# PixelClear/OclPathTracer

Hardware: NVIDIA B200
Metric: Mrays/sec (primary+secondary) (higher is better)
Workload: dtype f32

## Files before the change

oclpathtracer_b200/csrc/capi.cu:

```cuda
#include <cmath>
#include <cstdarg>
#include <cstdio>
#include <cstdlib>
#include <cstring>
#include <map>
#include <memory>
#include <string>
#include <vector>

#include "host_internal.h"
#include "pt_kernels.cuh"
#include "pt_wavefront.cuh"
#include "lbvh.cuh"

namespace ptb {

static thread_local char g_err[512] = "";

int fail(int code, const char* fmt, ...) {
    va_list ap;
    va_start(ap, fmt);
    vsnprintf(g_err, sizeof g_err, fmt, ap);
    va_end(ap);
    return code;
// ... 596 lines not shown
}

extern "C" int ptb_scene_mode_width(ptb_scene* s, int mode) {
    if (!s) return 0;
    const int c = mode_class(s, mode);
    return c == ptd::PTD_FLAT ? 1 : c == ptd::PTD_SMALL4 ? 4 : 2;
}

static ptd::SceneDev scene_dev(const ptb_scene* s, int cls) {
    ptd::SceneDev d;
    d.nodes = s->cls == ptd::PTD_LARGE ? reinterpret_cast<const float4*>(s->d_nodesq) : s->d_nodes;
    d.tris = s->d_tris; d.tris_orig = s->d_tris_orig; d.mats = s->d_mats;
    for (int a = 0; a < 3; ++a) { d.q_lo[a] = s->q_lo[a]; d.q_step[a] = s->q_step[a]; }
    d.n_nodes = s->n_nodes; d.n_tris = s->n_tris; d.n_mats = s->n_mats;
    if (cls == ptd::PTD_SMALL4 && s->cls == ptd::PTD_FLAT) {
        d.nodes = s->d_nodes4; d.n_nodes = int(s->built().nodes4.size());
        d.smem_nodes = s->built().smem_nodes4; d.small = 1; d.flat_n = 0; d.lstack = 0; d.ld256 = 0;
        d.stack_depth = 3 * s->built().depth4 + 1;
        return d;
    }
    const int cap = s->dev->tune[4] > 0 ? s->dev->tune[4] : 0;
    d.smem_nodes = s->small ? s->bfs_nodes : (s->bfs_nodes < cap ? s->bfs_nodes : cap);
    d.small = s->small ? 1 : 0;
    d.flat_n = 0;
    if (s->cls == ptd::PTD_FLAT) {
        d.flat_n = (int(s->built().flat.size()) + 1) & ~1;
        d.smem_nodes = 0;
    }
    d.stack_depth = s->width == 4 ? 3 * s->depth + 1 : s->depth + 1;
    d.lstack = (!s->small && s->dev->tune[2] != 2 && s->depth + 1 <= PTD_LSTACK_ENTRIES) ? 1 : 0;
    d.ld256 = s->dev->tune[8] == 1 ? 0 : 1;
    return d;
}


template <class K>
static int set_smem(K kernel, size_t smem, int block, int* per_sm = nullptr) {
    if (smem > 48 * 1024) CU_TRY(cudaFuncSetAttribute(kernel, cudaFuncAttributeMaxDynamicSharedMemorySize, (int)smem));
    int n = 0;
    CU_TRY(cudaOccupancyMaxActiveBlocksPerMultiprocessor(&n, kernel, block, smem));
    if (n < 1) n = 1;
    const size_t want = size_t(n) * (smem + 1024);
    int pct = (int)((want * 100 + 228 * 1024 - 1) / (228 * 1024));
    if (pct > 100) pct = 100;
    CU_TRY(cudaFuncSetAttribute(kernel, cudaFuncAttributePreferredSharedMemoryCarveout, pct));
    if (per_sm) *per_sm = n;
    return PTB_OK;
}

template <int MODE, bool BVH, int SMALL, bool STATS>
static int launch_mega_t(ptb_device* dev, const ptd::SceneDev& sc, const ptd::RenderArgs& a) {
    const int block = (a.tune[3] == 64 || a.tune[3] == 32) ? a.tune[3] : 128;
    if (MODE == PTB_MODE_PATH && a.tune[5] != 1) {
        const size_t smem = ptd::scene_smem_bytes(sc, BVH, SMALL, block) + (a.tune[9] > 0 ? size_t(a.tune[9]) * 1024 : 0);
        bool state_machine = BVH && SMALL == ptd::PTD_LARGE;
        if (a.tune[5] == 2) state_machine = false;
        if (a.tune[5] == 3) state_machine = BVH;
        const long long total = (long long)a.frames_in_batch * a.n_local;
        const long long need = (total + block - 1) / block;
        unsigned long long* work = dev->counters + 32;
        CU_TRY(cudaMemsetAsync(work, 0, sizeof(unsigned long long), dev->stream));
        int per_sm = 0;
        if constexpr (BVH) {
            if (state_machine) {
                ptd::SceneDev sc2 = sc;
                if (SMALL == ptd::PTD_LARGE && a.tune[4] == 0) sc2.smem_nodes = 0;
                const size_t smem2 = ptd::scene_smem_bytes(sc2, BVH, SMALL, block) + (a.tune[9] > 0 ? size_t(a.tune[9]) * 1024 : 0);
                auto k = ptd::k_path_sm<SMALL, STATS, 0, SMALL == ptd::PTD_LARGE ? 6 : 1>;
                if constexpr (SMALL == ptd::PTD_LARGE && !STATS) {
                    k = ptd::k_path_sm<SMALL, STATS, 8, 6>;
                    if (a.tune[12] == 1) k = ptd::k_path_sm<SMALL, STATS, 0, 6>;
                    if (a.tune[12] == 9) k = ptd::k_path_sm<SMALL, STATS, 9, 6>;
                    if (a.tune[14] == 1) k = ptd::k_path_sm<SMALL, STATS, 8, 1>;
                    if (a.tune[14] == 2) k = ptd::k_path_sm<SMALL, STATS, 8, 2>;
                    if (a.tune[14] == 4) k = ptd::k_path_sm<SMALL, STATS, 8, 4>;
                }
                if constexpr (SMALL == ptd::PTD_LARGE) {
                    if (a.tune[12] != 1 && a.tune[12] != 9 && a.tune[14] == 0 && sc2.lstack && sc2.smem_nodes == 0 && total < (1ll << 31) && a.tune[9] <= 0 && block == 128) {
                        auto k2 = ptd::k_path_sm2<STATS, STATS ? 0 : 11, 6>;
                        if constexpr (!STATS) {
                            if (a.tune[12] == 28) k2 = ptd::k_path_sm2<false, 8, 6>;
                            if (a.tune[12] == 29) k2 = ptd::k_path_sm2<false, 9, 6>;
                            if (a.tune[12] == 30) k2 = ptd::k_path_sm2<false, 10, 6>;
                            if (a.tune[12] == 32) k2 = ptd::k_path_sm2<false, 10, 4>;
                            if (a.tune[12] == 33) k2 = ptd::k_path_sm2<false, 10, 8>;
                        }
                        ptd::RenderArgs a2 = a;
                        if (a2.tune[0] <= 0) a2.tune[0] = 4;
                        if (a2.tune[10] <= 0) a2.tune[10] = 20;
                        if (a2.tune[11] <= 0) a2.tune[11] = 10;
                        const size_t sm2 = ptd::path_sm2_smem_bytes(block);
                        if (int rc = set_smem(k2, sm2, block, &per_sm)) return rc;
                        long long grid2 = (long long)per_sm * dev->prop.multiProcessorCount;
                        if (grid2 > need) grid2 = need;
                        k2<<<(unsigned)grid2, block, sm2, dev->stream>>>(sc2, a2, work);
                        CU_TRY(cudaGetLastError());
                        return PTB_OK;
                    }
                }
                if (int rc = set_smem(k, smem2, block, &per_sm)) return rc;
                if (a.tune[9] < 0 && -a.tune[9] < per_sm) per_sm = -a.tune[9];
                long long grid = (long long)per_sm * dev->prop.multiProcessorCount;
                if (grid > need) grid = need;
                k<<<(unsigned)grid, block, smem2, dev->stream>>>(sc2, a, work);
                CU_TRY(cudaGetLastError());
                return PTB_OK;
            }
        }
        auto k = ptd::k_mega_path_regen<BVH, SMALL, STATS>;
        if constexpr (BVH && SMALL == ptd::PTD_FLAT) if (a.tune[13] != 2) k = ptd::k_mega_path_regen<BVH, SMALL, STATS, true>;
        if (int rc = set_smem(k, smem, block, &per_sm)) return rc;
        long long grid = (long long)per_sm * dev->prop.multiProcessorCount;
        if (grid > need) grid = need;
        k<<<(unsigned)grid, block, smem, dev->stream>>>(sc, a, work);
        CU_TRY(cudaGetLastError());
        return PTB_OK;
    }
    const long long total = (long long)a.frames_in_batch * a.n_local;
    const unsigned grid = (unsigned)((total + block - 1) / block);
    const size_t smem = ptd::scene_smem_bytes(sc, BVH, SMALL, block);
    auto k = ptd::k_mega<MODE, BVH, SMALL, STATS>;
    if (int rc = set_smem(k, smem, block)) return rc;
    k<<<grid, block, smem, dev->stream>>>(sc, a);
    CU_TRY(cudaGetLastError());
    return PTB_OK;
}

template <int MODE>
static int launch_mega_m(ptb_device* dev, const ptd::SceneDev& sc, const ptd::RenderArgs& a, bool bvh, int small, bool stats) {
    using namespace ptd;
    if (!bvh && small == PTD_FLAT) small = PTD_SMALL4;
#define PTB_CASE(B, S, T) if (bvh == B && small == S && stats == T) return launch_mega_t<MODE, B, S, T>(dev, sc, a)
    PTB_CASE(true, PTD_FLAT, false); PTB_CASE(true, PTD_FLAT, true);
    PTB_CASE(true, PTD_SMALL4, false); PTB_CASE(true, PTD_SMALL4, true); PTB_CASE(true, PTD_LARGE, false); PTB_CASE(true, PTD_LARGE, true);
    PTB_CASE(false, PTD_SMALL4, false); PTB_CASE(false, PTD_SMALL4, true); PTB_CASE(false, PTD_LARGE, false); PTB_CASE(false, PTD_LARGE, true);
#undef PTB_CASE
    return fail(PTB_E_INVALID, "launch_mega: unreachable");
}

static int launch_mega(ptb_device* dev, int mode, const ptd::SceneDev& sc, const ptd::RenderArgs& a, bool bvh, int small, bool stats) {
    switch (mode) {
        case PTB_MODE_PRIMARY: return launch_mega_m<PTB_MODE_PRIMARY>(dev, sc, a, bvh, small, stats);
        case PTB_MODE_AO: return launch_mega_m<PTB_MODE_AO>(dev, sc, a, bvh, small, stats);
        case PTB_MODE_DIRECT: return launch_mega_m<PTB_MODE_DIRECT>(dev, sc, a, bvh, small, stats);
        case PTB_MODE_PATH: return launch_mega_m<PTB_MODE_PATH>(dev, sc, a, bvh, small, stats);
    }
    return fail(PTB_E_INVALID, "ptb_render: unknown mode %d", mode);
}


extern "C" void ptb_render_params_default(ptb_render_params* p) {
    if (!p) return;
    std::memset(p, 0, sizeof *p);
    p->width = 512; p->height = 512;
    p->first_frame = 0; p->n_frames = 1;
    p->mode = PTB_MODE_PATH;
    p->accum = PTB_ACCUM_REFERENCE;
    p->integrator = PTB_INTEGRATOR_AUTO;
    p->accel = PTB_ACCEL_BVH;
    p->max_depth = 16;
    p->ao_samples = 16;
    p->ao_max_dist = 2.0f;
    p->light_quad = 5;
    p->shard_index = 0; p->shard_count = 1; p->shard_block = 64;
}

extern "C" int ptb_render_local_pixels(const ptb_render_params* p) {
    if (!p) return 0;
// ... 1030 lines not shown
```

oclpathtracer_b200/csrc/pt_kernels.cuh:

```cuda
#pragma once

#include "pt_device.cuh"

namespace ptd {

enum { CTR_CLOSEST = 0, CTR_ANY = 1, CTR_NODES = 2, CTR_TESTS = 3, CTR_SAMPLES = 4, CTR_COUNT = 8 };

PTD_FI void flush_counter(unsigned long long* counters, int which, uint32_t v) {
    const uint32_t total = __reduce_add_sync(0xffffffffu, v);
    if ((threadIdx.x & 31) == 0 && total) atomicAdd(&counters[which], (unsigned long long)total);
}


PTD_FI uint32_t smem_u32(const void* p) { return (uint32_t)__cvta_generic_to_shared(p); }

PTD_FI void bulk_g2s(void* dst, const void* src, uint32_t bytes, void* mbar) {
    asm volatile("cp.async.bulk.shared::cluster.global.mbarrier::complete_tx::bytes [%0], [%1], %2, [%3];\n" ::"r"(
                     smem_u32(dst)),
                 "l"(src), "r"(bytes), "r"(smem_u32(mbar))
                 : "memory");
}

template <bool NODES, int SMALL, bool TRIS_BVH = NODES>
PTD_FI Ctx stage_scene(const SceneDev& sc, unsigned char* smem) {
// ... 36 lines not shown
                : "r"(smem_u32(mbar))
                : "memory");
        }
    }
    c.s_nodes = smem_u32(s_nodes);
    c.s_tris = smem_u32(s_tris);
    c.s_mats = smem_u32(s_mats);
    c.g_nodes = sc.nodes;
    c.g_tris = TRIS_BVH ? sc.tris : sc.tris_orig;
    c.g_mats = sc.mats;
    c.stride_bytes = blockDim.x * 4u;
    const uint32_t stack_bytes = (STACK && !sc.lstack) ? (uint32_t)sc.stack_depth * blockDim.x * 4u : 0u;
    c.s_stack64 = smem_u32(s_stack) + threadIdx.x * 8u;
    c.s_stack_ref = smem_u32(s_stack) + 2u * stack_bytes + threadIdx.x * 4u;
    c.s_scratch = smem_u32(s_stack) + 3u * stack_bytes + threadIdx.x * 4u;
    c.smem_nodes = sc.smem_nodes;
    c.n_tris = sc.n_tris;
    c.lstack = nullptr;
    c.ld256 = sc.ld256;
    c.flat_n = sc.flat_n;
    for (int k = 0; k < 3; ++k) { c.q_lo[k] = sc.q_lo[k]; c.q_step[k] = sc.q_step[k]; }
    c.s_coop = (BVH && SMALL == PTD_FLAT) ? smem_u32(s_stack) + (threadIdx.x >> 5) * (uint32_t)flat_coop_bytes_per_warp(sc.n_tris) : 0u;
    return c;
}

static inline size_t scene_smem_bytes(const SceneDev& sc, bool bvh, int small, int block, size_t scratch_per_thread = 0) {
    size_t b = 16;
    if (bvh) b += small == PTD_FLAT ? (size_t)sc.flat_n * 32 : (size_t)sc.smem_nodes * (small ? 128 : 32);
    if (small) b += (size_t)sc.n_tris * 48 + (size_t)sc.n_mats * 32;
    if (bvh && small != PTD_FLAT && !sc.lstack) b += (size_t)sc.stack_depth * block * 12;
    if (bvh && small == PTD_FLAT) b += (size_t)(block / 32) * (PTD_COOP_FIXED_BYTES + (((size_t)sc.n_tris * 64 + 15) & ~size_t(15)));
    return b + scratch_per_thread * block;
}


struct RenderArgs {
    int width, height;
    int first_frame;
    int frames_in_batch;
    int n_local;
    int max_depth, ao_samples;
    float ao_max_dist;
    int light_quad;
    float light_p1[3], light_ea[3], light_eb[3];
    float cam_inv_w, cam_inv_h, cam_aspect;
    float light_n[3], light_area;
    Shard shard;
    float4* samples;
    ptb_pixel_stats* stats;
    int stats_frame;
    unsigned long long* counters;
    int tune[16];
};

template <bool STATS>
struct SampleStats {
    int tri, quad;
    uint32_t t_bits, visits_primary, visits_secondary, count, id_hash, tri_tests;
};
template <>
struct SampleStats<false> {};

template <bool STATS>
PTD_FI void st_primary(SampleStats<STATS>& st, bool hit, const Hit& h, int quad, uint32_t visits) {
    if constexpr (STATS) {
        st.tri = hit ? h.idx : -1;
        st.quad = hit ? quad : -1;
        st.t_bits = hit ? __float_as_uint(h.t) : 0u;
        st.visits_primary = visits;
    }
}
template <bool STATS>
PTD_FI void st_secondary(SampleStats<STATS>& st, int tri, uint32_t visits) {
    if constexpr (STATS) {
        st.visits_secondary += visits;
        st.id_hash = st.id_hash * 31u + (uint32_t)(tri + 2);
    }
}

struct RayCount {
    uint32_t closest, any;
};

template <int SMALL, bool STATS>
PTD_FI bool path_after_hit(const Ctx& c, bool hit, const Hit& h, Ray& r, uint32_t& seed, V3& radiance, V3& mask, int i,
                           int max_depth, SampleStats<STATS>& st, uint32_t visits) {
    V3 p1, e1, e2; int idx = -1, quad = -1;
    if (hit) load_tri<SMALL>(c, h.pos, p1, e1, e2, idx, quad);
    if constexpr (STATS) {
        if (i == 0) st_primary(st, hit, h, quad, visits);
        else st_secondary(st, hit ? h.idx : -1, visits);
        st.count++;
    }
    if (!hit) {
        radiance = mk(radiance.x + mask.x * 0.45f, radiance.y + mask.y * 0.45f, radiance.z + mask.z * 0.45f);
        return false;
    }
    V3 p, n;
    hit_point_normal(e1, e2, r.o, r.d, h, p, n);
    V3 albedo, emissive; float roughness; int type;
    load_mat<SMALL>(c, quad, albedo, roughness, emissive, type);
    radiance = mk(radiance.x + mask.x * emissive.x * 3.0f, radiance.y + mask.y * emissive.y * 3.0f,
                  radiance.z + mask.z * emissive.z * 3.0f);
    if (i + 1 >= max_depth) return false;
    n = dot(n, r.d) < 0.0f ? n : mul(n, -1.0f);
    V3 wi = mk(0.0f, 0.0f, 0.0f);
    const V3 wo = neg(r.d);
    float pdf = 0.0f;
    const V3 color = brdf(wo, wi, pdf, n, albedo, roughness, type, seed);
    if (pdf <= 0.0f) return false;
    const float dw = dot(wi, n);
    mask = mk(mask.x * (color.x * dw / pdf), mask.y * (color.y * dw / pdf), mask.z * (color.z * dw / pdf));
    r = get_ray(add(p, mul(wi, 0.01f)), wi);
    return true;
}

template <bool BVH, int SMALL, bool STATS>
PTD_FI bool path_segment(const Ctx& c, Ray& r, uint32_t& seed, V3& radiance, V3& mask, int i, int max_depth,
                         SampleStats<STATS>& st, RayCount& rc, QueryStats& qs) {
    Hit h;
    const uint32_t v0 = qs.visits;
    const bool hit = q_closest<BVH, SMALL, STATS>(c, r.o, r.d, h, qs);
    rc.closest++;
    return path_after_hit<SMALL, STATS>(c, hit, h, r, seed, radiance, mask, i, max_depth, st, qs.visits - v0);
}

template <bool BVH, int SMALL, bool STATS>
PTD_FI V3 trace_rays(const Ctx& c, Ray r, uint32_t& seed, int max_depth, SampleStats<STATS>& st, RayCount& rc,
                     QueryStats& qs) {
    V3 radiance = mk(0.0f, 0.0f, 0.0f);
    V3 mask = mk(1.0f, 1.0f, 1.0f);
    for (int i = 0; i < max_depth; ++i)
        if (!path_segment<BVH, SMALL, STATS>(c, r, seed, radiance, mask, i, max_depth, st, rc, qs)) break;
    return mk(cl_max(radiance.x, 0.0f), cl_max(radiance.y, 0.0f), cl_max(radiance.z, 0.0f));
}

template <bool BVH, int SMALL, bool STATS>
PTD_FI V3 sample_primary(const Ctx& c, Ray r, SampleStats<STATS>& st, RayCount& rc, QueryStats& qs) {
    Hit h;
    const bool hit = q_closest<BVH, SMALL, STATS>(c, r.o, r.d, h, qs);
    rc.closest++;
    V3 p1, e1, e2; int idx = -1, quad = -1;
    if (hit) load_tri<SMALL>(c, h.pos, p1, e1, e2, idx, quad);
    st_primary(st, hit, h, quad, qs.visits);
    if constexpr (STATS) st.count = 1;
    if (!hit) return mk(0.45f, 0.45f, 0.45f);
    V3 albedo, emissive; float roughness; int type;
    load_mat<SMALL>(c, quad, albedo, roughness, emissive, type);
    return albedo;
}

template <bool BVH, int SMALL, bool STATS>
PTD_FI V3 sample_ao(const Ctx& c, Ray r, uint32_t& seed, int ns, float max_dist, SampleStats<STATS>& st,
                    RayCount& rc, QueryStats& qs) {
    Hit h;
    const bool hit = q_closest<BVH, SMALL, STATS>(c, r.o, r.d, h, qs);
    rc.closest++;
    V3 p1, e1, e2; int idx = -1, quad = -1;
    if (hit) load_tri<SMALL>(c, h.pos, p1, e1, e2, idx, quad);
    st_primary(st, hit, h, quad, qs.visits);
    if (!hit) return mk(1.0f, 1.0f, 1.0f);
    V3 p, n;
    hit_point_normal(e1, e2, r.o, r.d, h, p, n);
    n = dot(n, r.d) < 0.0f ? n : mul(n, -1.0f);
    uint32_t open = 0;
    const Frame fr = make_frame(n);
    for (int k = 0; k < ns; ++k) {
        const V3 wi = sample_hemisphere_cosine(n, fr, seed);
        const Ray s = get_ray(add(p, mul(wi, 0.01f)), wi);
        Hit b;
        const uint32_t v0 = qs.visits;
        const bool occ = q_any<BVH, SMALL, STATS>(c, s.o, s.d, max_dist, b, qs);
        rc.any++;
        st_secondary(st, occ ? b.idx : -1, qs.visits - v0);
        if (!occ) open++;
    }
    if constexpr (STATS) st.count = open;
    const float v = (float)open / (float)ns;
    return mk(v, v, v);
}

template <bool BVH, int SMALL, bool STATS>
PTD_FI V3 sample_direct(const Ctx& c, const RenderArgs& a, Ray r, uint32_t& seed, SampleStats<STATS>& st,
                        RayCount& rc, QueryStats& qs) {
    Hit h;
    const bool hit = q_closest<BVH, SMALL, STATS>(c, r.o, r.d, h, qs);
    rc.closest++;
    V3 p1, e1, e2; int idx = -1, quad = -1;
    if (hit) load_tri<SMALL>(c, h.pos, p1, e1, e2, idx, quad);
    st_primary(st, hit, h, quad, qs.visits);
    if (!hit) return mk(0.45f, 0.45f, 0.45f);
    V3 albedo, emissive; float roughness; int type;
    load_mat<SMALL>(c, quad, albedo, roughness, emissive, type);
    V3 p, n;
    hit_point_normal(e1, e2, r.o, r.d, h, p, n);
    V3 col = mk(1.0f * emissive.x * 3.0f, 1.0f * emissive.y * 3.0f, 1.0f * emissive.z * 3.0f);
    n = dot(n, r.d) < 0.0f ? n : mul(n, -1.0f);
// ... 272 lines not shown
                        else state = ST_SHADE;
                    }
                }
                continue;
            }
            if (!n_node || n_shade >= thr_shade) break;
            if (state == ST_NODE) {
                if constexpr (SMALL == PTD_FLAT) {
                    tm = flat_boxes<STATS>(c, r.o, r.d, 1e20f, qs);
                    state = tm ? ST_LEAF : ST_SHADE;
                } else {
                    bool more;
                    if (SMALL == PTD_LARGE && fast_nodes) {
                        more = node_step2_bf<STATS>(c, rp, best_t, cur, sp, qs);
#pragma unroll
                        for (int rep = 1; rep < NSTEP; ++rep)
                            if (more && cur >= 0) more = node_step2_bf<STATS>(c, rp, best_t, cur, sp, qs);
                    }
                    else more = node_step<false, SMALL, STATS>(c, rp, best_t, cur, sp, qs);
                    state = !more ? ST_SHADE : cur >= 0 ? ST_NODE : ST_LEAF;
                }
            }
        }
        if (state == ST_SHADE) {
            Hit h;
            const bool hit = best_idx >= 0;
            h.t = best_t; h.u = best_u; h.v = best_v; h.pos = best_pos; h.idx = best_idx;
            rc.closest++;
            const bool more = path_after_hit<SMALL, STATS>(c, hit, h, r, seed, radiance, mask, depth, a.max_depth, st, qs.visits - visits0);
            ++depth;
            if (!more || depth >= a.max_depth) {
                a.samples[slot] = make_float4(cl_max(radiance.x, 0.0f), cl_max(radiance.y, 0.0f), cl_max(radiance.z, 0.0f), 1.0f);
                if constexpr (STATS) {
                    if (a.stats && frame == a.stats_frame) {
                        uint4* dst = reinterpret_cast<uint4*>(a.stats + li);
                        dst[0] = make_uint4((uint32_t)st.tri, (uint32_t)st.quad, st.t_bits, st.visits_primary);
                        dst[1] = make_uint4(st.visits_secondary, st.count, st.id_hash, qs.tests - tests0);
                    }
                }
                state = exhausted ? ST_DONE : ST_REGEN;
            } else {
                begin_query();
            }
        }
        const unsigned m_regen = __ballot_sync(0xffffffffu, state == ST_REGEN);
        const unsigned m_walk = __ballot_sync(0xffffffffu, (state & (ST_NODE | ST_LEAF)) != 0u);
        const uint32_t n_regen = __popc(m_regen);
        if (n_regen && (n_regen >= thr_regen || !m_walk)) {
            const int leader = __ffs(m_regen) - 1;
            unsigned long long base = 0;
            if ((int)lane == leader) base = atomicAdd(work_counter, (unsigned long long)n_regen);
            base = __shfl_sync(0xffffffffu, base, leader);
            if ((long long)base + (long long)n_regen >= total) exhausted = true;
            if (state == ST_REGEN) {
                slot = (long long)base + __popc(m_regen & ((1u << lane) - 1u));
                if (slot >= total) {
                    state = ST_DONE;
                } else {
                    const int fi = (int)(slot / a.n_local);
                    li = (int)(slot - (long long)fi * a.n_local);
                    const int gid = gid_of_local(a.shard, li);
                    frame = a.first_frame + fi;
                    seed = (uint32_t)gid + hash_uint32((uint32_t)frame);
                    r = generate_ray(gid % a.width, gid / a.width, CamScale{a.cam_inv_w, a.cam_inv_h, a.cam_aspect}, seed);
                    radiance = mk(0.f, 0.f, 0.f);
                    mask = mk(1.f, 1.f, 1.f);
                    depth = 0;
                    st = SampleStats<STATS>{};
                    tests0 = qs.tests;
                    begin_query();
                }
            }
        } else if (!m_walk) {
            break;
        }
    }
    flush_counter(a.counters, CTR_CLOSEST, rc.closest);
    if (STATS) {
        flush_counter(a.counters, CTR_NODES, qs.visits);
        flush_counter(a.counters, CTR_TESTS, qs.tests);
    }
}

enum { PK_OX = 0, PK_OY, PK_OZ, PK_DX, PK_DY, PK_DZ, PK_U, PK_V, PK_POS, PK_IDX, PK_RX, PK_RY, PK_RZ, PK_MX, PK_MY, PK_MZ, PK_SEED, PK_SLOT, PK_DEPTH, PK_FIELDS };
static inline size_t path_sm2_smem_bytes(int block) { return 16 + (size_t)PK_FIELDS * block * 4; }

template <bool STATS, int MINB, int NSTEP>
__global__ void __launch_bounds__(128, MINB) k_path_sm2(const SceneDev sc, const RenderArgs a, unsigned long long* work_counter) {
    extern __shared__ __align__(16) unsigned char smem[];
    Ctx c = stage_scene<true, PTD_LARGE>(sc, smem);
    uint2 lstack_mem[PTD_LSTACK_ENTRIES + 1];
    c.lstack = lstack_mem + 1;
    uint32_t pk = smem_u32(smem) + 16u + threadIdx.x * 4u;
    asm volatile("" : "+r"(pk));
    constexpr uint32_t fstride = 128u * 4u;
#define PKL(f) lds32(pk + (uint32_t)(f) * fstride)
#define PKLF(f) __uint_as_float(lds32(pk + (uint32_t)(f) * fstride))
#define PKS(f, v) sts32(pk + (uint32_t)(f) * fstride, (uint32_t)(v))
#define PKSF(f, v) sts32(pk + (uint32_t)(f) * fstride, __float_as_uint(v))
    const uint32_t total = (uint32_t)((long long)a.frames_in_batch * a.n_local);
    const unsigned lane = threadIdx.x & 31u;
    const uint32_t thr_regen = (uint32_t)a.tune[0], thr_shade = (uint32_t)a.tune[10], thr_leaf = (uint32_t)a.tune[11];
    RayCount rc{0u, 0u};
    QueryStats qs{0u, 0u};
    uint32_t state = ST_REGEN;
    bool exhausted = false;
    int li = 0, frame = 0;
    uint32_t tests0 = 0, visits0 = 0;
    RayPre rp{mk(0.f, 0.f, 0.f), mk(0.f, 0.f, 0.f), {0u, 0u, 0u}};
    float best_t = 1e20f;
    int cur = 0, sp = 0;
    SampleStats<STATS> st{};
    auto begin_query = [&](const Ray& r) {
        visits0 = qs.visits;
        best_t = 1e20f;
        PKS(PK_IDX, -1);
        rp = ray_pre<PTD_LARGE>(c, r.o, r.d);
        cur = 0; sp = 0;
        state = ST_NODE;
    };
    for (;;) {
        for (;;) {
            const uint32_t cnt = __reduce_add_sync(0xffffffffu, state);
            const uint32_t n_node = (cnt >> 8) & 255u, n_leaf = (cnt >> 16) & 255u, n_shade = cnt >> 24;
            if (n_leaf >= thr_leaf || (n_leaf && !n_node)) {
                if (state == ST_LEAF) {
                    const int k = (int)((uint32_t)(~cur) >> 3);
                    V3 p1, e1, e2; int idx, quad;
                    load_tri<PTD_LARGE>(c, k, p1, e1, e2, idx, quad);
                    const V3 o = mk(PKLF(PK_OX), PKLF(PK_OY), PKLF(PK_OZ)), d = mk(PKLF(PK_DX), PKLF(PK_DY), PKLF(PK_DZ));
                    float t, u, v;
                    if (STATS) qs.tests++;
                    if (mt_core(o, d, p1, e1, e2, t, u, v)) {
                        bool take = t < best_t;
                        if (t == best_t) { const int bi = (int)PKL(PK_IDX); take = bi >= 0 && idx < bi; }
                        if (take) {
                            best_t = t;
                            PKSF(PK_U, u); PKSF(PK_V, v); PKS(PK_POS, k); PKS(PK_IDX, idx);
                        }
                    }
                    const uint32_t code = (uint32_t)(~cur);
                    if (code & 7u) cur = (int)~(((code >> 3) + 1u) << 3 | ((code & 7u) - 1u));
                    else if (stack_pop<false>(c, sp, cur, best_t)) state = cur >= 0 ? ST_NODE : ST_LEAF;
                    else state = ST_SHADE;
                }
                continue;
            }
            if (!n_node || n_shade >= thr_shade) break;
            if (state == ST_NODE) {
                bool more = node_step2_bf<STATS>(c, rp, best_t, cur, sp, qs);
#pragma unroll
                for (int rep = 1; rep < NSTEP; ++rep)
                    if (more && cur >= 0) more = node_step2_bf<STATS>(c, rp, best_t, cur, sp, qs);
                state = !more ? ST_SHADE : cur >= 0 ? ST_NODE : ST_LEAF;
            }
        }
        if (state == ST_SHADE) {
            Ray r{mk(PKLF(PK_OX), PKLF(PK_OY), PKLF(PK_OZ)), mk(PKLF(PK_DX), PKLF(PK_DY), PKLF(PK_DZ))};
            V3 radiance = mk(PKLF(PK_RX), PKLF(PK_RY), PKLF(PK_RZ)), mask = mk(PKLF(PK_MX), PKLF(PK_MY), PKLF(PK_MZ));
            uint32_t seed = PKL(PK_SEED);
            int depth = (int)PKL(PK_DEPTH);
            Hit h;
            h.idx = (int)PKL(PK_IDX);
            const bool hit = h.idx >= 0;
            h.t = best_t; h.u = PKLF(PK_U); h.v = PKLF(PK_V); h.pos = (int)PKL(PK_POS);
            rc.closest++;
            const bool more = path_after_hit<PTD_LARGE, STATS>(c, hit, h, r, seed, radiance, mask, depth, a.max_depth, st, qs.visits - visits0);
            ++depth;
            if (!more || depth >= a.max_depth) {
                a.samples[PKL(PK_SLOT)] = make_float4(cl_max(radiance.x, 0.0f), cl_max(radiance.y, 0.0f), cl_max(radiance.z, 0.0f), 1.0f);
                if constexpr (STATS) {
                    if (a.stats && frame == a.stats_frame) {
                        uint4* dst = reinterpret_cast<uint4*>(a.stats + li);
                        dst[0] = make_uint4((uint32_t)st.tri, (uint32_t)st.quad, st.t_bits, st.visits_primary);
                        dst[1] = make_uint4(st.visits_secondary, st.count, st.id_hash, qs.tests - tests0);
                    }
                }
                state = exhausted ? ST_DONE : ST_REGEN;
            } else {
                PKSF(PK_OX, r.o.x); PKSF(PK_OY, r.o.y); PKSF(PK_OZ, r.o.z); PKSF(PK_DX, r.d.x); PKSF(PK_DY, r.d.y); PKSF(PK_DZ, r.d.z);
                PKSF(PK_RX, radiance.x); PKSF(PK_RY, radiance.y); PKSF(PK_RZ, radiance.z);
                PKSF(PK_MX, mask.x); PKSF(PK_MY, mask.y); PKSF(PK_MZ, mask.z);
                PKS(PK_SEED, seed); PKS(PK_DEPTH, depth);
                begin_query(r);
            }
        }
        const unsigned m_regen = __ballot_sync(0xffffffffu, state == ST_REGEN);
        const unsigned m_walk = __ballot_sync(0xffffffffu, (state & (ST_NODE | ST_LEAF)) != 0u);
        const uint32_t n_regen = __popc(m_regen);
        if (n_regen && (n_regen >= thr_regen || !m_walk)) {
            const int leader = __ffs(m_regen) - 1;
            unsigned long long base = 0;
            if ((int)lane == leader) base = atomicAdd(work_counter, (unsigned long long)n_regen);
            base = __shfl_sync(0xffffffffu, base, leader);
            if (base + n_regen >= (unsigned long long)total) exhausted = true;
            if (state == ST_REGEN) {
                const unsigned long long slot = base + __popc(m_regen & ((1u << lane) - 1u));
                if (slot >= (unsigned long long)total) {
                    state = ST_DONE;
                } else {
                    const int fi = (int)(slot / (unsigned)a.n_local);
                    const int l = (int)(slot - (unsigned long long)fi * (unsigned)a.n_local);
                    const int gid = gid_of_local(a.shard, l);
                    li = l; frame = a.first_frame + fi;
                    uint32_t seed = (uint32_t)gid + hash_uint32((uint32_t)(a.first_frame + fi));
                    const Ray r = generate_ray(gid % a.width, gid / a.width, CamScale{a.cam_inv_w, a.cam_inv_h, a.cam_aspect}, seed);
                    PKSF(PK_OX, r.o.x); PKSF(PK_OY, r.o.y); PKSF(PK_OZ, r.o.z); PKSF(PK_DX, r.d.x); PKSF(PK_DY, r.d.y); PKSF(PK_DZ, r.d.z);
                    PKSF(PK_RX, 0.0f); PKSF(PK_RY, 0.0f); PKSF(PK_RZ, 0.0f); PKSF(PK_MX, 1.0f); PKSF(PK_MY, 1.0f); PKSF(PK_MZ, 1.0f);
                    PKS(PK_SEED, seed); PKS(PK_SLOT, (uint32_t)slot); PKS(PK_DEPTH, 0);
                    st = SampleStats<STATS>{};
                    tests0 = qs.tests;
                    begin_query(r);
                }
            }
        } else if (!m_walk) {
            break;
        }
    }
#undef PKL
#undef PKLF
#undef PKS
#undef PKSF
    flush_counter(a.counters, CTR_CLOSEST, rc.closest);
    if (STATS) {
        flush_counter(a.counters, CTR_NODES, qs.visits);
        flush_counter(a.counters, CTR_TESTS, qs.tests);
    }
}


PTD_FI V3 gamma_correct(V3 v) {
    const float g = 1.0f / 2.2f;
    return mk(det_pow(v.x, g), det_pow(v.y, g), det_pow(v.z, g));
}
PTD_FI V3 read_from_gamma(V3 v) {
    return mk(det_pow(v.x, 2.2f), det_pow(v.y, 2.2f), det_pow(v.z, 2.2f));
}

struct ResolveArgs {
    const float4* samples;
    int n_local, frames_in_batch, first_frame;
    int accum;
    int first_batch, last_batch;
    int total_frames;
    float4* sum;
    float4* frame;
    int gather, n_peers;
    Shard shard;
    float4* peers[PTB_MAX_PEERS];
};

PTD_FI void resolve_store(const ResolveArgs& a, size_t at, float4 v) {
    a.frame[at] = v;
    for (int k = 0; k < a.n_peers; ++k) a.peers[k][at] = v;
}

__global__ void __launch_bounds__(256) k_resolve(const ResolveArgs a) {
    const int li = blockIdx.x * blockDim.x + threadIdx.x;
    if (li >= a.n_local) return;
    const size_t at = a.gather ? (size_t)gid_of_local(a.shard, li) : (size_t)li;
    if (a.accum == PTB_ACCUM_REFERENCE) {
        float4 cur = a.frame[at];
        V3 state = xyz(cur);
        float w = cur.w;
        for (int fi = 0; fi < a.frames_in_batch; ++fi) {
            const V3 col = xyz(a.samples[(size_t)fi * a.n_local + li]);
            const int f = a.first_frame + fi;
// ... 133 lines not shown
```

Baseline: 4896.

## Keep path state and ray precompute in shared memory during shading and traversal

Makes the shading routine generic over a state accessor so the persistent wavefront kernel can read and write ray, radiance, mask and seed fields directly in the per-thread shared-memory columns instead of loading them all into registers. The ray precompute (inverse direction, sign bits) is also moved into shared memory and reloaded before each traversal step. The goal is lower register pressure and higher occupancy. The cost is more shared-memory traffic per step and per shade, plus a larger shared-memory footprint per block. Two tuning variants are removed.

```diff
diff --git a/oclpathtracer_b200/csrc/capi.cu b/oclpathtracer_b200/csrc/capi.cu
--- a/oclpathtracer_b200/csrc/capi.cu
+++ b/oclpathtracer_b200/csrc/capi.cu
@@ -702,8 +702,6 @@
                             if (a.tune[12] == 28) k2 = ptd::k_path_sm2<false, 8, 6>;
                             if (a.tune[12] == 29) k2 = ptd::k_path_sm2<false, 9, 6>;
                             if (a.tune[12] == 30) k2 = ptd::k_path_sm2<false, 10, 6>;
-                            if (a.tune[12] == 32) k2 = ptd::k_path_sm2<false, 10, 4>;
-                            if (a.tune[12] == 33) k2 = ptd::k_path_sm2<false, 10, 8>;
                         }
                         ptd::RenderArgs a2 = a;
                         if (a2.tune[0] <= 0) a2.tune[0] = 4;
diff --git a/oclpathtracer_b200/csrc/pt_kernels.cuh b/oclpathtracer_b200/csrc/pt_kernels.cuh
--- a/oclpathtracer_b200/csrc/pt_kernels.cuh
+++ b/oclpathtracer_b200/csrc/pt_kernels.cuh
@@ -142,9 +142,28 @@
     uint32_t closest, any;
 };
 
-template <int SMALL, bool STATS>
-PTD_FI bool path_after_hit(const Ctx& c, bool hit, const Hit& h, Ray& r, uint32_t& seed, V3& radiance, V3& mask, int i,
-                           int max_depth, SampleStats<STATS>& st, uint32_t visits) {
+struct PathRegs {
+    Ray& r;
+    uint32_t& seed;
+    V3& radiance;
+    V3& mask;
+    V3 hp;
+    PTD_FI V3 o() const { return r.o; }
+    PTD_FI V3 d() const { return r.d; }
+    PTD_FI uint32_t rng() const { return seed; }
+    PTD_FI V3 rad() const { return radiance; }
+    PTD_FI V3 msk() const { return mask; }
+    PTD_FI V3 hit_point() const { return hp; }
+    PTD_FI void set_rng(uint32_t v) { seed = v; }
+    PTD_FI void set_rad(V3 v) { radiance = v; }
+    PTD_FI void set_msk(V3 v) { mask = v; }
+    PTD_FI void set_hit_point(V3 v) { hp = v; }
+    PTD_FI void set_ray(const Ray& v) { r = v; }
+};
+
+template <int SMALL, bool STATS, class PS>
+PTD_FI bool path_after_hit(const Ctx& c, bool hit, const Hit& h, PS& ps, int i, int max_depth, SampleStats<STATS>& st,
+                           uint32_t visits) {
     V3 p1, e1, e2; int idx = -1, quad = -1;
     if (hit) load_tri<SMALL>(c, h.pos, p1, e1, e2, idx, quad);
     if constexpr (STATS) {
@@ -153,26 +172,41 @@
         st.count++;
     }
     if (!hit) {
-        radiance = mk(radiance.x + mask.x * 0.45f, radiance.y + mask.y * 0.45f, radiance.z + mask.z * 0.45f);
+        const V3 radiance = ps.rad(), mask = ps.msk();
+        ps.set_rad(mk(radiance.x + mask.x * 0.45f, radiance.y + mask.y * 0.45f, radiance.z + mask.z * 0.45f));
         return false;
     }
     V3 p, n;
-    hit_point_normal(e1, e2, r.o, r.d, h, p, n);
+    hit_point_normal(e1, e2, ps.o(), ps.d(), h, p, n);
+    ps.set_hit_point(p);
     V3 albedo, emissive; float roughness; int type;
     load_mat<SMALL>(c, quad, albedo, roughness, emissive, type);
-    radiance = mk(radiance.x + mask.x * emissive.x * 3.0f, radiance.y + mask.y * emissive.y * 3.0f,
-                  radiance.z + mask.z * emissive.z * 3.0f);
+    {
+        const V3 radiance = ps.rad(), mask = ps.msk();
+        ps.set_rad(mk(radiance.x + mask.x * emissive.x * 3.0f, radiance.y + mask.y * emissive.y * 3.0f,
+                      radiance.z + mask.z * emissive.z * 3.0f));
+    }
     if (i + 1 >= max_depth) return false;
-    n = dot(n, r.d) < 0.0f ? n : mul(n, -1.0f);
+    const V3 d = ps.d();
+    n = dot(n, d) < 0.0f ? n : mul(n, -1.0f);
     V3 wi = mk(0.0f, 0.0f, 0.0f);
-    const V3 wo = neg(r.d);
+    const V3 wo = neg(d);
     float pdf = 0.0f;
+    uint32_t seed = ps.rng();
     const V3 color = brdf(wo, wi, pdf, n, albedo, roughness, type, seed);
+    ps.set_rng(seed);
     if (pdf <= 0.0f) return false;
     const float dw = dot(wi, n);
-    mask = mk(mask.x * (color.x * dw / pdf), mask.y * (color.y * dw / pdf), mask.z * (color.z * dw / pdf));
-    r = get_ray(add(p, mul(wi, 0.01f)), wi);
+    const V3 mask = ps.msk();
+    ps.set_msk(mk(mask.x * (color.x * dw / pdf), mask.y * (color.y * dw / pdf), mask.z * (color.z * dw / pdf)));
+    ps.set_ray(get_ray(add(ps.hit_point(), mul(wi, 0.01f)), wi));
     return true;
+}
+template <int SMALL, bool STATS>
+PTD_FI bool path_after_hit(const Ctx& c, bool hit, const Hit& h, Ray& r, uint32_t& seed, V3& radiance, V3& mask, int i,
+                           int max_depth, SampleStats<STATS>& st, uint32_t visits) {
+    PathRegs ps{r, seed, radiance, mask, {}};
+    return path_after_hit<SMALL, STATS>(c, hit, h, ps, i, max_depth, st, visits);
 }
 
 template <bool BVH, int SMALL, bool STATS>
@@ -611,8 +645,31 @@
     }
 }
 
-enum { PK_OX = 0, PK_OY, PK_OZ, PK_DX, PK_DY, PK_DZ, PK_U, PK_V, PK_POS, PK_IDX, PK_RX, PK_RY, PK_RZ, PK_MX, PK_MY, PK_MZ, PK_SEED, PK_SLOT, PK_DEPTH, PK_FIELDS };
+enum { PK_OX = 0, PK_OY, PK_OZ, PK_DX, PK_DY, PK_DZ, PK_U, PK_V, PK_POS, PK_IDX, PK_RX, PK_RY, PK_RZ, PK_MX, PK_MY, PK_MZ, PK_SEED, PK_SLOT, PK_DEPTH,
+       PK_AX, PK_AY, PK_AZ, PK_BX, PK_BY, PK_BZ, PK_SN0, PK_SN1, PK_SN2, PK_FIELDS };
 static inline size_t path_sm2_smem_bytes(int block) { return 16 + (size_t)PK_FIELDS * block * 4; }
+constexpr uint32_t PK_STRIDE = 128u * 4u;
+
+struct PathCol {
+    uint32_t pk;
+    Ray r;
+    PTD_FI float ldf(int f) const { return __uint_as_float(lds32(pk + (uint32_t)f * PK_STRIDE)); }
+    PTD_FI void stf(int f, float v) const { sts32(pk + (uint32_t)f * PK_STRIDE, __float_as_uint(v)); }
+    PTD_FI V3 o() const { return mk(ldf(PK_OX), ldf(PK_OY), ldf(PK_OZ)); }
+    PTD_FI V3 d() const { return mk(ldf(PK_DX), ldf(PK_DY), ldf(PK_DZ)); }
+    PTD_FI uint32_t rng() const { return lds32(pk + PK_SEED * PK_STRIDE); }
+    PTD_FI V3 rad() const { return mk(ldf(PK_RX), ldf(PK_RY), ldf(PK_RZ)); }
+    PTD_FI V3 msk() const { return mk(ldf(PK_MX), ldf(PK_MY), ldf(PK_MZ)); }
+    PTD_FI V3 hit_point() const { return o(); }
+    PTD_FI void set_rng(uint32_t v) { sts32(pk + PK_SEED * PK_STRIDE, v); }
+    PTD_FI void set_rad(V3 v) { stf(PK_RX, v.x); stf(PK_RY, v.y); stf(PK_RZ, v.z); }
+    PTD_FI void set_msk(V3 v) { stf(PK_MX, v.x); stf(PK_MY, v.y); stf(PK_MZ, v.z); }
+    PTD_FI void set_hit_point(V3 v) { stf(PK_OX, v.x); stf(PK_OY, v.y); stf(PK_OZ, v.z); }
+    PTD_FI void set_ray(const Ray& v) {
+        r = v;
+        stf(PK_OX, v.o.x); stf(PK_OY, v.o.y); stf(PK_OZ, v.o.z); stf(PK_DX, v.d.x); stf(PK_DY, v.d.y); stf(PK_DZ, v.d.z);
+    }
+};
 
 template <bool STATS, int MINB, int NSTEP>
 __global__ void __launch_bounds__(128, MINB) k_path_sm2(const SceneDev sc, const RenderArgs a, unsigned long long* work_counter) {
@@ -622,11 +679,10 @@
     c.lstack = lstack_mem + 1;
     uint32_t pk = smem_u32(smem) + 16u + threadIdx.x * 4u;
     asm volatile("" : "+r"(pk));
-    constexpr uint32_t fstride = 128u * 4u;
-#define PKL(f) lds32(pk + (uint32_t)(f) * fstride)
-#define PKLF(f) __uint_as_float(lds32(pk + (uint32_t)(f) * fstride))
-#define PKS(f, v) sts32(pk + (uint32_t)(f) * fstride, (uint32_t)(v))
-#define PKSF(f, v) sts32(pk + (uint32_t)(f) * fstride, __float_as_uint(v))
+#define PKL(f) lds32(pk + (uint32_t)(f) * PK_STRIDE)
+#define PKLF(f) __uint_as_float(lds32(pk + (uint32_t)(f) * PK_STRIDE))
+#define PKS(f, v) sts32(pk + (uint32_t)(f) * PK_STRIDE, (uint32_t)(v))
+#define PKSF(f, v) sts32(pk + (uint32_t)(f) * PK_STRIDE, __float_as_uint(v))
     const uint32_t total = (uint32_t)((long long)a.frames_in_batch * a.n_local);
     const unsigned lane = threadIdx.x & 31u;
     const uint32_t thr_regen = (uint32_t)a.tune[0], thr_shade = (uint32_t)a.tune[10], thr_leaf = (uint32_t)a.tune[11];
@@ -636,7 +692,6 @@
     bool exhausted = false;
     int li = 0, frame = 0;
     uint32_t tests0 = 0, visits0 = 0;
-    RayPre rp{mk(0.f, 0.f, 0.f), mk(0.f, 0.f, 0.f), {0u, 0u, 0u}};
     float best_t = 1e20f;
     int cur = 0, sp = 0;
     SampleStats<STATS> st{};
@@ -644,7 +699,9 @@
         visits0 = qs.visits;
         best_t = 1e20f;
         PKS(PK_IDX, -1);
-        rp = ray_pre<PTD_LARGE>(c, r.o, r.d);
+        const RayPre q = ray_pre<PTD_LARGE>(c, r.o, r.d);
+        PKSF(PK_AX, q.a.x); PKSF(PK_AY, q.a.y); PKSF(PK_AZ, q.a.z); PKSF(PK_BX, q.b.x); PKSF(PK_BY, q.b.y); PKSF(PK_BZ, q.b.z);
+        PKS(PK_SN0, q.sn[0]); PKS(PK_SN1, q.sn[1]); PKS(PK_SN2, q.sn[2]);
         cur = 0; sp = 0;
         state = ST_NODE;
     };
@@ -677,6 +734,7 @@
             }
             if (!n_node || n_shade >= thr_shade) break;
             if (state == ST_NODE) {
+                const RayPre rp{mk(PKLF(PK_AX), PKLF(PK_AY), PKLF(PK_AZ)), mk(PKLF(PK_BX), PKLF(PK_BY), PKLF(PK_BZ)), {PKL(PK_SN0), PKL(PK_SN1), PKL(PK_SN2)}};
                 bool more = node_step2_bf<STATS>(c, rp, best_t, cur, sp, qs);
 #pragma unroll
                 for (int rep = 1; rep < NSTEP; ++rep)
@@ -685,18 +743,16 @@
             }
         }
         if (state == ST_SHADE) {
-            Ray r{mk(PKLF(PK_OX), PKLF(PK_OY), PKLF(PK_OZ)), mk(PKLF(PK_DX), PKLF(PK_DY), PKLF(PK_DZ))};
-            V3 radiance = mk(PKLF(PK_RX), PKLF(PK_RY), PKLF(PK_RZ)), mask = mk(PKLF(PK_MX), PKLF(PK_MY), PKLF(PK_MZ));
-            uint32_t seed = PKL(PK_SEED);
-            int depth = (int)PKL(PK_DEPTH);
             Hit h;
             h.idx = (int)PKL(PK_IDX);
             const bool hit = h.idx >= 0;
             h.t = best_t; h.u = PKLF(PK_U); h.v = PKLF(PK_V); h.pos = (int)PKL(PK_POS);
+            const int depth = (int)PKL(PK_DEPTH);
             rc.closest++;
-            const bool more = path_after_hit<PTD_LARGE, STATS>(c, hit, h, r, seed, radiance, mask, depth, a.max_depth, st, qs.visits - visits0);
-            ++depth;
-            if (!more || depth >= a.max_depth) {
+            PathCol ps{pk, {}};
+            const bool more = path_after_hit<PTD_LARGE, STATS>(c, hit, h, ps, depth, a.max_depth, st, qs.visits - visits0);
+            if (!more || depth + 1 >= a.max_depth) {
+                const V3 radiance = ps.rad();
                 a.samples[PKL(PK_SLOT)] = make_float4(cl_max(radiance.x, 0.0f), cl_max(radiance.y, 0.0f), cl_max(radiance.z, 0.0f), 1.0f);
                 if constexpr (STATS) {
                     if (a.stats && frame == a.stats_frame) {
@@ -707,11 +763,8 @@
                 }
                 state = exhausted ? ST_DONE : ST_REGEN;
             } else {
-                PKSF(PK_OX, r.o.x); PKSF(PK_OY, r.o.y); PKSF(PK_OZ, r.o.z); PKSF(PK_DX, r.d.x); PKSF(PK_DY, r.d.y); PKSF(PK_DZ, r.d.z);
-                PKSF(PK_RX, radiance.x); PKSF(PK_RY, radiance.y); PKSF(PK_RZ, radiance.z);
-                PKSF(PK_MX, mask.x); PKSF(PK_MY, mask.y); PKSF(PK_MZ, mask.z);
-                PKS(PK_SEED, seed); PKS(PK_DEPTH, depth);
-                begin_query(r);
+                PKS(PK_DEPTH, depth + 1);
+                begin_query(ps.r);
             }
         }
         const unsigned m_regen = __ballot_sync(0xffffffffu, state == ST_REGEN);
```

After: 5153 (median of 6 runs). +5.2%, better.
